# jsdjayanga/kmer-counter

Measured on NVIDIA B200. Metric: k-mers counted/s at k=31, higher is better.
Workload: dtype u64

## Files before the change

kmer-counter_b200/csrc/kc_super.cu:

```cuda
#include <math.h>
#include <stdlib.h>

#include "kc_internal.h"
#include "kc_super.cuh"

namespace kc {

namespace {

constexpr uint32_t kNoBin = 0xffffffffu;
constexpr int kSwThreads = 256;
constexpr int kSwMaxSeg = 18;
constexpr int kNb1Max = 1024;
constexpr int kRsBins = 2048;

template <uint32_t X> struct ILog2 { static constexpr uint32_t v = 1 + ILog2<(X >> 1)>::v; };
template <> struct ILog2<1> { static constexpr uint32_t v = 0; };

__host__ __device__ __forceinline__ uint32_t mmer_hash(uint32_t mm) {
    uint32_t h = mm * 0x9E3779B1u;
    h ^= h >> 15;
    h *= 0x85EBCA6Bu;
    return h;
}
__device__ __forceinline__ uint32_t bin_of_min(uint32_t mn, uint32_t n_bins) {
    return __umulhi(mn * 0xC2B2AE35u, n_bins);
}

struct SwScatterParams {
    ExtractParams ep;
    uint32_t m, w, nh, nh_stride, seg_len, segs_per_read, cmax, span;
    uint32_t h_off, bin_off, bits_off;
    uint32_t n_bins, bin_cap;
    uint64_t ovf_cap;
    uint32_t *cursor;
    uint8_t *bins;
    uint8_t *ovf;
    unsigned long long *sc;
};

template <int W, bool CANON>
__global__ void __launch_bounds__(kSwThreads) sw_scatter_kernel(SwScatterParams q) {
    const ExtractParams &p = q.ep;
    extern __shared__ __align__(128) uint8_t smem[];
    const uint32_t stage_bytes = p.stage_bytes;
    uint8_t *stage0 = smem;
    uint64_t *enc = reinterpret_cast<uint64_t *>(smem + p.enc_off);
    uint8_t *enc_b = reinterpret_cast<uint8_t *>(enc);
    const uint32_t enc_row = p.nw + 1;
    uint8_t *bad4 = smem + p.bad_off;
    uint8_t *flag = smem + p.flag_off;
    uint64_t *bars = reinterpret_cast<uint64_t *>(smem + p.bar_off);
    uint32_t *hh = reinterpret_cast<uint32_t *>(smem + q.h_off);
    uint32_t *bid = reinterpret_cast<uint32_t *>(smem + q.bin_off);
    uint32_t *seg_st = reinterpret_cast<uint32_t *>(smem + q.bits_off);
    uint32_t *seg_bd = seg_st + p.tile_reads * q.segs_per_read;
    __shared__ uint32_t s_nstart;
    const uint32_t tid = threadIdx.x, lane = tid & 31;

    if (tid == 0) {
        s_nstart = 0;
        mbar_init(&bars[0], 1);
        mbar_init(&bars[1], 1);
        mbar_fence_init();
    }
    for (uint32_t i = tid; i < p.tile_reads * enc_row; i += kSwThreads) enc[i] = 0;
    for (uint32_t i = tid; i < p.tile_reads; i += kSwThreads) flag[i] = 0;
    __syncthreads();

    auto tile_reads_of = [&](uint32_t t) -> uint32_t {
        uint64_t first = (uint64_t)t * p.tile_reads;
        uint64_t left = p.n_reads - first;
        return left < p.tile_reads ? (uint32_t)left : p.tile_reads;
    };
    auto issue_load = [&](uint32_t t, uint32_t s) {
        uint32_t bytes = tile_reads_of(t) * p.L;
        const uint8_t *src = p.reads + (uint64_t)t * p.tile_reads * p.L;
        uint8_t *dst = stage0 + s * stage_bytes;
        if ((bytes & 15u) == 0) {
            if (tid == 0) {
                asm volatile("fence.proxy.async.shared::cta;" ::: "memory");
                mbar_expect_tx(&bars[s], bytes);
                tma_load_1d(dst, src, bytes, &bars[s]);
            }
        } else {
            for (uint32_t i = tid; i < bytes; i += kSwThreads) dst[i] = src[i];
        }
    };

    uint32_t phase_bits = 0, stage = 0;
    unsigned long long invalid_local = 0, windows_local = 0, records_local = 0;
    const uint32_t mmask = q.m >= 16 ? 0xffffffffu : ((1u << (2 * q.m)) - 1u);
    const uint32_t mshift = 64 - 2 * q.m;
    const uint32_t ng = (q.nh + 7) >> 3;

    uint32_t tile = blockIdx.x;
    if (tile < p.n_tiles) issue_load(tile, 0);

    for (; tile < p.n_tiles; tile += gridDim.x) {
        const uint32_t next = tile + gridDim.x;
        if (next < p.n_tiles) issue_load(next, stage ^ 1);
        const uint32_t nreads = tile_reads_of(tile);
        if (((nreads * p.L) & 15u) == 0) {
            mbar_wait(&bars[stage], (phase_bits >> stage) & 1u);
            phase_bits ^= 1u << stage;
        } else {
            __syncthreads();
        }
        const uint8_t *src_tile = stage0 + stage * stage_bytes;

        encode_tile(p, src_tile, nreads, enc_b, bad4, flag);
        __syncthreads();
        if (tid == 0) s_nstart = 0;

        for (uint32_t g = tid; g < nreads * ng; g += kSwThreads) {
            const uint32_t r = g / ng, j0 = (g - r * ng) * 8;
            const uint32_t wi = j0 >> 5, sh = (j0 & 31u) * 2u;
            const uint64_t *e = enc + r * enc_row;
            const uint64_t a = wi <= p.nw ? e[wi] : 0ull;
            const uint64_t b = wi + 1 <= p.nw ? e[wi + 1] : 0ull;
            const uint64_t x = sh ? ((a << sh) | (b >> (64 - sh))) : a;
            uint32_t *row = hh + r * q.nh_stride + j0;
            if constexpr (CANON) {
#pragma unroll
                for (uint32_t i = 0; i < 8; i++) {
                    const uint32_t mm = (uint32_t)(x >> (mshift - 2 * i)) & mmask;
                    uint32_t r = __brev(mm);
                    r = ((r >> 1) & 0x55555555u) | ((r & 0x55555555u) << 1);
                    if (j0 + i < q.nh) row[i] = mmer_hash(min(mm, (r >> (32 - 2 * q.m)) ^ mmask));
                }
            } else {
#pragma unroll
                for (uint32_t i = 0; i < 8; i++)
                    if (j0 + i < q.nh) row[i] = mmer_hash((uint32_t)(x >> (mshift - 2 * i)) & mmask);
            }
        }
        __syncthreads();

        const uint32_t n_seg = nreads * q.segs_per_read;
        for (uint32_t sg = tid; sg < n_seg; sg += kSwThreads) {
            const uint32_t r = sg / q.segs_per_read;
            const uint32_t p0 = (sg - r * q.segs_per_read) * q.seg_len;
            if (p0 >= p.nk) { seg_st[sg] = 0; seg_bd[sg] = 0; continue; }
            const uint32_t s = min(q.seg_len, p.nk - p0);
            const uint32_t lb = p0 > 0 ? 1u : 0u;
            const uint32_t se = s + lb;
            const uint32_t *g = hh + r * q.nh_stride + p0 - lb;
            uint32_t S[kSwMaxSeg];
            S[kSwMaxSeg - 1] = 0xffffffffu;
#pragma unroll
            for (int i = kSwMaxSeg - 2; i >= 0; i--) {
                const uint32_t v = (uint32_t)i + 1 < se ? g[i] : 0xffffffffu;
                S[i] = min(v, S[i + 1]);
            }
            uint32_t core = 0xffffffffu;
            for (uint32_t t = se - 1; t < q.w; t++) core = min(core, g[t]);
            uint32_t pm = 0xffffffffu;
            const bool check = flag[r] != 0;
            uint32_t *brow = bid + r * p.nk + p0 - lb;
            uint32_t prev = kNoBin, stm = 0, bdm = 0;
#pragma unroll
            for (uint32_t i = 0; i < (uint32_t)kSwMaxSeg; i++) {
                if (i < se) {
                    const uint32_t mn = min(min(S[i], core), pm);
                    const bool valid = check ? kmer_window_valid(bad4 + r * p.nb4, p0 - lb + i, p.k) : true;
                    const uint32_t b = valid ? bin_of_min(mn, q.n_bins) : kNoBin;
                    if (i >= lb) {
                        if (!valid) invalid_local++;
                        brow[i] = b;
                        const uint32_t st = (valid && b != prev) ? 1u : 0u;
                        stm |= st << (i - lb);
                        bdm |= (st | (valid ? 0u : 1u)) << (i - lb);
                    }
                    prev = b;
                    if (i + 1 < se) pm = min(pm, g[q.w + i]);
                }
            }
            seg_st[sg] = stm;
            seg_bd[sg] = bdm;
        }
        __syncthreads();

        uint32_t *list = hh;
        for (uint32_t base = 0; base < n_seg; base += kSwThreads) {
            const uint32_t sg = base + tid;
            uint32_t stm = sg < n_seg ? seg_st[sg] : 0u;
            const uint32_t cnt = __popc(stm);
            uint32_t incl = cnt;
#pragma unroll
            for (int o = 1; o < 32; o <<= 1) {
                const uint32_t t = __shfl_up_sync(0xffffffffu, incl, o);
                if (lane >= (uint32_t)o) incl += t;
            }
            uint32_t off = 0;
            if (lane == 31 && incl) off = atomicAdd(&s_nstart, incl);
            off = __shfl_sync(0xffffffffu, off, 31) + incl - cnt;
            while (stm) {
                const uint32_t i = __ffs(stm) - 1;
                stm &= stm - 1;
                list[off++] = (sg << 5) | i;
            }
        }
        __syncthreads();
        const uint32_t n_start = s_nstart;
        for (uint32_t en = tid; en < n_start; en += kSwThreads) {
            const uint32_t ent = list[en];
            const uint32_t sg = ent >> 5, wi0 = ent & 31u;
            const uint32_t r = sg / q.segs_per_read, si = sg - r * q.segs_per_read;
            const uint32_t pos = si * q.seg_len + wi0;
            uint32_t end = p.nk;
            {
                uint32_t mk = seg_bd[sg] & ~(0xffffffffu >> (31 - wi0));
                uint32_t sj = si;
                while (mk == 0 && ++sj < q.segs_per_read) mk = seg_bd[r * q.segs_per_read + sj];
                if (mk) end = min(p.nk, sj * q.seg_len + (uint32_t)__ffs(mk) - 1);
            }
            const uint32_t len = end - pos;
            const uint32_t b = bid[r * p.nk + pos];
            const uint64_t *e = enc + r * enc_row;
            for (uint32_t q0 = 0; q0 < len; q0 += q.cmax) {
                const uint32_t idx = atomicAdd(&q.cursor[b], 1u);
                const uint32_t c = min(q.cmax, len - q0);
                const uint32_t wi = (pos + q0) >> 5, sh = ((pos + q0) & 31u) * 2u;
                uint64_t ew[2 * W + 1];
#pragma unroll
                for (int t = 0; t < 2 * W + 1; t++) ew[t] = wi + t <= p.nw ? e[wi + t] : 0ull;
                uint64_t rec[2 * W];
#pragma unroll
                for (int t = 0; t < 2 * W; t++) rec[t] = sh ? ((ew[t] << sh) | (ew[t + 1] >> (64 - sh))) : ew[t];
                const uint32_t nbases = q.span + c - 1;
#pragma unroll
                for (int t = 0; t < 2 * W; t++) {
                    const int keep = (int)nbases - 32 * t;
                    if (keep <= 0) rec[t] = 0;
                    else if (keep < 32) rec[t] &= ~0ull << (64 - 2 * keep);
                }
                rec[2 * W - 1] = (rec[2 * W - 1] & ~0xffull) | c;
                ulonglong2 *dst = nullptr;
                if (idx < q.bin_cap) {
                    dst = reinterpret_cast<ulonglong2 *>(q.bins) + ((uint64_t)b * q.bin_cap + idx) * W;
                } else {
                    const unsigned long long oi = atomicAdd(&q.sc[SW_OVF], 1ull);
                    if (oi < q.ovf_cap) dst = reinterpret_cast<ulonglong2 *>(q.ovf) + oi * W;
                    else atomicOr(&q.sc[SW_FAIL], 1ull);
                }
                if (dst) {
#pragma unroll
                    for (int t = 0; t < W; t++) dst[t] = make_ulonglong2(rec[2 * t], rec[2 * t + 1]);
                }
                windows_local += c;
                records_local++;
            }
        }
        for (uint32_t i = tid; i < nreads; i += kSwThreads) flag[i] = 0;
        __syncthreads();
        stage ^= 1;
    }
#pragma unroll
    for (int o = 16; o > 0; o >>= 1) {
        invalid_local += __shfl_xor_sync(0xffffffffu, invalid_local, o);
        windows_local += __shfl_xor_sync(0xffffffffu, windows_local, o);
        records_local += __shfl_xor_sync(0xffffffffu, records_local, o);
    }
    if (lane == 0) {
        if (invalid_local) atomicAdd(&q.sc[SW_INVALID], invalid_local);
        if (windows_local) atomicAdd(&q.sc[SW_WINDOWS], windows_local);
        if (records_local) atomicAdd(&q.sc[SW_RECORDS], records_local);
    }
}

template <int W> __device__ __forceinline__ bool key_all_ones(const Key<W> &k) {
    uint64_t a = ~0ull;
#pragma unroll
    for (int i = 0; i < W; i++) a &= k.w[i];
    return a == ~0ull;
}
template <int W> __device__ __forceinline__ bool key_any_word_ones(const Key<W> &k) {
    bool r = false;
#pragma unroll
    for (int i = 0; i < W; i++) r = r || (k.w[i] == ~0ull);
    return r;
}
template <int W> __device__ __forceinline__ void key_set_ones(Key<W> &k) {
#pragma unroll
    for (int i = 0; i < W; i++) k.w[i] = ~0ull;
}
__device__ __forceinline__ Key<1> slot_claim(Key<1> *slot, const Key<1> &k) {
    Key<1> o;
    o.w[0] = atomicCAS(reinterpret_cast<unsigned long long *>(slot), ~0ull, (unsigned long long)k.w[0]);
    return o;
}
__device__ __forceinline__ Key<2> slot_claim(Key<2> *slot, const Key<2> &k) {
    Key<2> o;
    const uint32_t a = smem_u32(slot);
    asm volatile(
        "{\n"
        ".reg .b128 c, n, o;\n"
        "mov.b128 c, {%3, %3};\n"
        "mov.b128 n, {%4, %5};\n"
        "atom.shared.cas.b128 o, [%2], c, n;\n"
        "mov.b128 {%0, %1}, o;\n"
        "}\n"
        : "=l"(o.w[0]), "=l"(o.w[1])
        : "r"(a), "l"(~0ull), "l"(k.w[0]), "l"(k.w[1])
        : "memory");
    return o;
}
template <int W> __device__ __forceinline__ uint32_t key_hash(const Key<W> &k) {
    uint32_t x = (uint32_t)k.w[0] ^ (uint32_t)(k.w[0] >> 29);
    if constexpr (W > 1) x ^= ((uint32_t)k.w[W - 1] ^ (uint32_t)(k.w[W - 1] >> 31)) * 0x85EBCA6Bu;
    return x * 0x9E3779B1u;
}
__device__ __forceinline__ uint32_t pass_hash(uint32_t h) { return (h ^ (h >> 15)) * 0x2C1B3C6Du; }

enum {
    SWP_UNIT = 0,
    SWP_DEDUP,
    SWP_SCAN,
    SWP_OPEN,
    SWP_INSERT,
    SWP_DRAIN,
    SWP_ROUND_END,
    SWP_EMIT,
    SWP_PHASES,
    SWP_QUEUED = SWP_PHASES,
    SWP_DRAIN_PROBES,
    SWP_WARPS,
    SWP_TOTAL,
    SWP_SLOTS
};
#ifdef KC_SW_PROFILE
__device__ unsigned long long g_sw_prof[SWP_SLOTS];
#define SWP_DECL                                                                                      \
    __shared__ unsigned long long s_prof[THREADS / 32][SWP_SLOTS];                                    \
    if (lane == 0)                                                                                    \
        for (int i_ = 0; i_ < SWP_SLOTS; i_++) s_prof[warp][i_] = 0;                                  \
    const long long swp_t0 = clock64();                                                               \
    long long swp_t = swp_t0
#define SWP_MARK(ph)                                                                                  \
    do {                                                                                              \
        const long long t_ = clock64();                                                               \
        if (lane == 0) s_prof[warp][ph] += (unsigned long long)(t_ - swp_t);                          \
        swp_t = t_;                                                                                   \
    } while (0)
#define SWP_ADD(c, v) atomicAdd(&s_prof[warp][c], (unsigned long long)(v))
#define SWP_ADD_ACTIVE(c)                                                                             \
    do {                                                                                              \
        const uint32_t am_ = __activemask();                                                          \
        if (lane == (uint32_t)__ffs(am_) - 1) SWP_ADD(c, __popc(am_));                                \
    } while (0)
#define SWP_FLUSH()                                                                                   \
    do {                                                                                              \
        __syncwarp();                                                                                 \
        if (lane == 0) {                                                                              \
            s_prof[warp][SWP_WARPS] = 1;                                                              \
            s_prof[warp][SWP_TOTAL] = (unsigned long long)(clock64() - swp_t0);                       \
            for (int i_ = 0; i_ < SWP_SLOTS; i_++) atomicAdd(&g_sw_prof[i_], s_prof[warp][i_]);       \
        }                                                                                             \
    } while (0)
#else
#define SWP_DECL do {} while (0)
#define SWP_MARK(ph) do {} while (0)
#define SWP_ADD(c, v) do {} while (0)
#define SWP_ADD_ACTIVE(c) do {} while (0)
#define SWP_FLUSH() do {} while (0)
#endif

struct SwCountParams {
    uint32_t n_src;
    const uint32_t *src_cursor[8];
    const uint8_t *src_bins[8];
    const unsigned long long *src_sc[8];
    uint32_t bin_begin;
    const uint8_t *ovf;
    uint32_t n_bins, bin_cap, ovf_slice;
    uint64_t ovf_cap;
    uint64_t last_mask;
    uint64_t *d_keys;
    uint32_t *d_counts;
    uint64_t d_cap;
    uint32_t *hist1;
    int shift1, nb1;
    int add_phantom;
    unsigned long long *sc;
};

template <int W, int THREADS, int TSLOTS, int RPT, bool CANON = false>
__global__ void __launch_bounds__(THREADS) sw_count_kernel(SwCountParams p) {
    constexpr int RB = THREADS * RPT;
    extern __shared__ __align__(16) uint8_t cs_smem[];
    Key<W> *tk = reinterpret_cast<Key<W> *>(cs_smem);
    ulonglong2 *recs = reinterpret_cast<ulonglong2 *>(tk + TSLOTS);
    uint32_t *tc = reinterpret_cast<uint32_t *>(recs + RB * W);
    uint32_t *s_start = tc + TSLOTS;
    uint32_t *s_hist = s_start + THREADS;
    constexpr int kQueue = RPT > 1 ? 64 : 96;
    Key<W> *queue = reinterpret_cast<Key<W> *>(s_hist + kNb1Max);
    uint32_t *queue_m = reinterpret_cast<uint32_t *>(queue + (THREADS / 32) * kQueue);
    constexpr bool DEDUP = (W == 1);
    constexpr int RT = DEDUP ? (RPT > 1 ? RB : 2 * RB) : 1;
    ulonglong2 *rt_keys = reinterpret_cast<ulonglong2 *>(queue_m + (THREADS / 32) * kQueue);
    uint32_t *rt_mult = reinterpret_cast<uint32_t *>(rt_keys + RT);
    uint32_t *rec_mult = rt_mult + RT;
    __shared__ uint32_t s_unit, s_m, s_ones, s_abort;
    __shared__ unsigned long long s_base;
    __shared__ uint32_t s_warp[THREADS / 32];
    const uint32_t tid = threadIdx.x, lane = tid & 31, warp = tid >> 5;
    constexpr uint32_t kLimit = TSLOTS / 4 * 3;
    constexpr uint32_t hshift = 32 - ILog2<(uint32_t)TSLOTS>::v;
    [[maybe_unused]] const uint32_t rc_sh = CANON ? rc_shift_of(p.last_mask) : 0u;

    {
        Key<W> empty;
        key_set_ones<W>(empty);
        for (uint32_t i = tid; i < (uint32_t)TSLOTS; i += THREADS) { tk[i] = empty; tc[i] = 0; }
        for (uint32_t i = tid; i < (uint32_t)p.nb1; i += THREADS) s_hist[i] = 0;
        if constexpr (DEDUP)
            for (uint32_t i = tid; i < (uint32_t)RT; i += THREADS) { rt_keys[i] = make_ulonglong2(~0ull, ~0ull); rt_mult[i] = 0; }
        if (tid == 0) { s_m = 0; s_ones = 0; s_abort = 0; }
    }
    unsigned long long n_ovf = p.sc[SW_OVF];
// ... 1228 lines not shown
inline uint64_t round512(uint64_t b) { return (b + 511) & ~511ull; }

constexpr int kFinCapSmall = 2048, kFinCapLarge = 4096;
constexpr int kFinCapWide = 1024;

}

static void plan_layout(SuperPlan &pl, bool ext_e);

bool super_plan(uint32_t k, uint32_t L, uint32_t flags, uint64_t max_windows, uint32_t occ_per_bin, SuperPlan *out,
                double record_headroom, uint64_t distinct_hint, bool ext_e) {
    if (k == 0 || k > 64 || L < k || L > 4096) return false;
    if (flags & kPlanCanonical) flags |= kPlanStrict;
    const bool strict = (flags & kPlanStrict) != 0;
    SuperPlan pl{};
    pl.flags = flags & (kPlanStrict | kPlanCanonical);
    pl.W = (int)((k + 31) / 32);
    pl.k = k;
    pl.L = L;
    const uint32_t mm = k % 32;
    const bool masked = strict ? (mm != 0) : (mm >= 1 && mm <= 28);
    pl.span = masked ? k : 32u * pl.W;
    pl.last_mask = masked ? (~0ull << (64 - 2 * mm)) : ~0ull;
    if (pl.span < 22) return false;
    pl.nk = L - k + 1;
    pl.cmax = 32u * pl.W - 3;
    if (max_windows == 0) max_windows = 1;
    if (occ_per_bin == 0) {
        occ_per_bin = 8192;
        if (distinct_hint && distinct_hint < max_windows) {
            const double per_key = (double)max_windows / (double)distinct_hint;
            const double occ = 2200.0 * per_key;
            if (occ < 8192.0) occ_per_bin = occ < 1024.0 ? 1024u : ((uint32_t)occ + 255u) & ~255u;
        }
    }
    uint64_t nb = (max_windows + occ_per_bin - 1) / occ_per_bin;
    if (nb < 8) nb = 8;
    if (nb > (1ull << 24)) nb = 1ull << 24;
    pl.n_bins = (uint32_t)nb;
    pl.m = 12;
    while (pl.m < 16 && pl.m + 8 < pl.span && (1ull << (2 * pl.m)) < 192ull * pl.n_bins) pl.m++;
    pl.w = pl.span - pl.m + 1;
    pl.nh = pl.nk + pl.w - 1;
    pl.nh_stride = (pl.nh + 8) | 1u;
    pl.seg_len = pl.w - 1 < (uint32_t)kSwMaxSeg - 1 ? pl.w - 1 : (uint32_t)kSwMaxSeg - 1;
    pl.segs_per_read = (pl.nk + pl.seg_len - 1) / pl.seg_len;
    pl.seg_len = (pl.nk + pl.segs_per_read - 1) / pl.segs_per_read;
    const double rho = 2.0 / (pl.w + 1) + 1.2 / pl.nk + 1.0 / pl.cmax * 0.25;
    const double est_total = (double)max_windows * rho;
    const double per_bin = est_total / (double)pl.n_bins;
    pl.bin_cap = (uint32_t)(per_bin * (1.0 + 90.0 / sqrt((double)occ_per_bin))) + 64;
    pl.bin_cap = (pl.bin_cap + 3) & ~3u;
    pl.ovf_cap = (uint64_t)(est_total * 0.6) + 8192;
    if (pl.ovf_cap < max_windows / 16) pl.ovf_cap = max_windows / 16;
    pl.ovf_slice = 4096;
    const uint64_t d_base = distinct_hint && distinct_hint < max_windows ? distinct_hint + distinct_hint / 8 + 4096 : max_windows;
    pl.d_cap = d_base + (uint64_t)((double)d_base * record_headroom) + (record_headroom > 0 ? 8192 : 0);
    if (pl.d_cap > (1ull << 32) - 2) pl.d_cap = (1ull << 32) - 2;
    if (pl.d_cap < 1024) pl.d_cap = 1024;
    pl.fin_cap = pl.d_cap > (uint64_t)kSuperMaxSub * (kFinCapSmall * 7 / 10) ? kFinCapLarge : kFinCapSmall;
    pl.sub_target = pl.fin_cap * 7 / 10;
    if (const char *v = getenv("KC_SW_SUB_TARGET")) {
        const int t = atoi(v);
        if (t > 0) pl.sub_target = (uint32_t)t;
    }
    const int sig = pl.W == 1 ? (masked ? (int)(2 * mm) : 64) : 64;
    pl.b1 = sig < 10 ? sig : 10;
    plan_layout(pl, ext_e);
    *out = pl;
    return true;
}

static void plan_layout(SuperPlan &pl, bool ext_e) {
    uint64_t o = 0;
    auto take = [&](uint64_t bytes) { uint64_t r = o; o += round512(bytes); return r; };
    const uint64_t rec_bytes = 16ull * pl.W;
    pl.off_cursor = take((uint64_t)pl.n_bins * 4);
    pl.off_hist1 = take((kNb1Max + 8) * 4);
    pl.off_hist2 = take((uint64_t)(2 * kSuperMaxSub + 8) * 4);
    pl.off_base1 = take((kNb1Max + 8) * 4);
    pl.off_cur1 = take((kNb1Max + 8) * 4);
    pl.off_base2 = take((uint64_t)(kSuperMaxSub + 8) * 4);
    pl.off_cur2 = take((uint64_t)(kSuperMaxSub + 8) * 4);
    pl.off_mout = take((uint64_t)(kSuperMaxSub + 8) * 4);
    pl.off_off = take((uint64_t)(kSuperMaxSub + 8) * 4);
    pl.off_plan = take(sizeof(SuperPlanDev));
    pl.off_x = take(sizeof(XDev));
    pl.off_sc = take(SW_COUNT * 8);
    pl.off_h2m = take((uint64_t)(kSuperMaxSub + 8) * 4);
    pl.off_big = take((uint64_t)(kSuperMaxSub + 8) * 4);
    pl.off_bigoff = take((uint64_t)(kSuperMaxSub + 8) * 4);
    pl.off_bins = take((uint64_t)pl.n_bins * pl.bin_cap * rec_bytes);
    pl.off_ovf = take(pl.ovf_cap * rec_bytes);
    pl.off_dk = take(pl.d_cap * 8 * pl.W + 64);
    pl.off_dc = take(pl.d_cap * 4 + 64);
    pl.ext_e = ext_e;
    pl.ext_ek = nullptr;
    pl.ext_ec = nullptr;
    pl.off_ek = pl.off_ec = o;
    if (!ext_e) {
        pl.off_ek = take(pl.d_cap * 8 * pl.W + 64);
        pl.off_ec = take(pl.d_cap * 4 + 64);
    }
    pl.ws_bytes = o;
}

bool place_plan(uint32_t k, bool strict, uint64_t n_records, SuperPlan *out) {
    if (k == 0 || k > 128 || n_records == 0 || n_records > (1ull << 32) - 2) return false;
    SuperPlan pl{};
    pl.W = (int)((k + 31) / 32);
    pl.k = k;
    const uint32_t mm = k % 32;
    const bool masked = strict ? (mm != 0) : (mm >= 1 && mm <= 28);
    pl.span = masked ? k : 32u * pl.W;
    pl.last_mask = masked ? (~0ull << (64 - 2 * mm)) : ~0ull;
    pl.n_bins = 8;
    pl.d_cap = n_records < 1024 ? 1024 : n_records;
    pl.fin_cap = pl.W >= 3 && n_records <= (uint64_t)kSuperMaxSub * (kFinCapWide * 7 / 10) ? kFinCapWide : kFinCapSmall;
    pl.sub_target = pl.fin_cap * 7 / 10;
    if (const char *v = getenv("KC_SW_SUB_TARGET")) {
        const int t = atoi(v);
        if (t > 0) pl.sub_target = (uint32_t)t;
    }
    const int sig = pl.W == 1 ? (masked ? (int)(2 * mm) : 64) : 64;
    pl.b1 = sig < 10 ? sig : 10;
    plan_layout(pl, false);
    *out = pl;
    return true;
}

namespace {
template <class T> T *at(void *ws, uint64_t off) { return reinterpret_cast<T *>(static_cast<uint8_t *>(ws) + off); }
uint64_t *ek_of(const SuperPlan &pl, void *ws) { return pl.ext_e ? pl.ext_ek : at<uint64_t>(ws, pl.off_ek); }
uint32_t *ec_of(const SuperPlan &pl, void *ws) { return pl.ext_e ? pl.ext_ec : at<uint32_t>(ws, pl.off_ec); }
}

cudaError_t super_reset(const SuperPlan &pl, void *ws, unsigned long long *d_sc, cudaStream_t s) {
    cudaError_t e;
    if ((e = cudaMemsetAsync(ws, 0, pl.off_base1, s)) != cudaSuccess) return e;
    return cudaMemsetAsync(d_sc, 0, SW_COUNT * 8, s);
}

template <int W>
static cudaError_t super_scatter_w(const SuperPlan &pl, const void *d_reads, uint64_t n_reads, void *ws,
                                   unsigned long long *d_sc, int n_sms, cudaStream_t s) {
    static int tile_bytes = -1;
    if (tile_bytes < 0) { const char *v = getenv("KC_SW_STAGE"); tile_bytes = v ? atoi(v) : 4800; }
    SwScatterParams q{};
    if (!extract_plan(d_reads, n_reads, pl.L, pl.k, pl.flags, &d_sc[SW_INVALID], &q.ep, (uint32_t)tile_bytes))
        return cudaErrorInvalidValue;
    if (q.ep.n_tiles == 0) return cudaSuccess;
    q.m = pl.m; q.w = pl.w; q.nh = pl.nh; q.nh_stride = pl.nh_stride;
    q.seg_len = pl.seg_len; q.segs_per_read = pl.segs_per_read; q.cmax = pl.cmax; q.span = pl.span;
    q.h_off = (q.ep.smem_total + 15u) & ~15u;
    q.bin_off = q.h_off + q.ep.tile_reads * pl.nh_stride * 4;
    q.bits_off = q.bin_off + q.ep.tile_reads * pl.nk * 4;
    const uint32_t smem = q.bits_off + 2 * q.ep.tile_reads * pl.segs_per_read * 4;
    if (smem > 200 * 1024) return cudaErrorInvalidValue;
    q.n_bins = pl.n_bins; q.bin_cap = pl.bin_cap; q.ovf_cap = pl.ovf_cap;
    q.cursor = at<uint32_t>(ws, pl.off_cursor);
    q.bins = at<uint8_t>(ws, pl.off_bins);
    q.ovf = at<uint8_t>(ws, pl.off_ovf);
    q.sc = d_sc;
    auto kern = (pl.flags & kPlanCanonical) ? sw_scatter_kernel<W, true> : sw_scatter_kernel<W, false>;
    cudaError_t e = cudaFuncSetAttribute(kern, cudaFuncAttributeMaxDynamicSharedMemorySize, (int)smem);
    if (e != cudaSuccess) return e;
    int per_sm = 1;
    cudaOccupancyMaxActiveBlocksPerMultiprocessor(&per_sm, kern, kSwThreads, smem);
    per_sm = per_sm < 1 ? 1 : (per_sm > 6 ? 6 : per_sm);
    uint32_t grid = (uint32_t)n_sms * per_sm;
    if (grid > q.ep.n_tiles) grid = q.ep.n_tiles;
    kern<<<grid, kSwThreads, smem, s>>>(q);
    return cudaGetLastError();
}

static bool super_scatter_fits(const SuperPlan &pl) {
    ExtractParams ep;
    if (!extract_plan(nullptr, 16, pl.L, pl.k, 0u, nullptr, &ep, 6400)) return false;
    const uint64_t smem = ((ep.smem_total + 15u) & ~15u) + (uint64_t)ep.tile_reads * pl.nh_stride * 4 +
                          (uint64_t)ep.tile_reads * pl.nk * 4 + 2ull * ep.tile_reads * pl.segs_per_read * 4;
    return smem <= 200 * 1024;
}

cudaError_t super_scatter(const SuperPlan &pl, const void *d_reads, uint64_t n_reads, void *ws,
                          unsigned long long *d_sc, int n_sms, cudaStream_t s) {
    if (pl.W == 1) return super_scatter_w<1>(pl, d_reads, n_reads, ws, d_sc, n_sms, s);
    if (pl.W == 2) return super_scatter_w<2>(pl, d_reads, n_reads, ws, d_sc, n_sms, s);
    return cudaErrorInvalidValue;
}

template <int W, int THREADS, int TSLOTS, int RPT = 2, bool CANON = false>
static cudaError_t launch_count(const SwCountParams &cp, int n_sms, cudaStream_t s) {
    const uint32_t RB = THREADS * RPT, RT = W == 1 ? (RPT > 1 ? RB : 2 * RB) : 1;
    const uint32_t smem = TSLOTS * (8 * W + 4) + RB * 16 * W + THREADS * 4 + kNb1Max * 4 +
                          (THREADS / 32) * (RPT > 1 ? 64 : 96) * (8 * W + 4) + RT * 20 + RB * 4 + 64;
    auto kern = sw_count_kernel<W, THREADS, TSLOTS, RPT, CANON>;
    cudaError_t e = cudaFuncSetAttribute(kern, cudaFuncAttributeMaxDynamicSharedMemorySize, (int)smem);
    if (e != cudaSuccess) return e;
    int per_sm = 1;
    cudaOccupancyMaxActiveBlocksPerMultiprocessor(&per_sm, kern, THREADS, smem);
    if (per_sm < 1) per_sm = 1;
    kern<<<(uint32_t)n_sms * per_sm, THREADS, smem, s>>>(cp);
    return cudaGetLastError();
}

template <int W>
static cudaError_t super_count_bins_w(const SuperPlan &pl, bool add_phantom, void *ws, unsigned long long *d_sc, int n_sms,
                                      cudaStream_t s, void *const *peer_ws = nullptr, uint32_t rank = 0,
                                      uint32_t n_ranks = 1) {
    cudaError_t e;
    SwCountParams cp{};
    const uint32_t n_src = peer_ws ? n_ranks : 1u;
    cp.n_src = n_src;
    for (uint32_t i = 0; i < n_src; i++) {
        void *w = peer_ws ? peer_ws[i] : ws;
        cp.src_cursor[i] = at<uint32_t>(w, pl.off_cursor);
        cp.src_bins[i] = at<uint8_t>(w, pl.off_bins);
        cp.src_sc[i] = peer_ws ? at<unsigned long long>(w, pl.off_sc) : d_sc;
    }
    cp.bin_begin = peer_ws ? (uint32_t)((uint64_t)pl.n_bins * rank / n_ranks) : 0u;
    cp.n_bins = peer_ws ? (uint32_t)((uint64_t)pl.n_bins * (rank + 1) / n_ranks) - cp.bin_begin : pl.n_bins;
    cp.ovf = at<uint8_t>(ws, pl.off_ovf);
    cp.bin_cap = pl.bin_cap; cp.ovf_slice = pl.ovf_slice; cp.ovf_cap = pl.ovf_cap;
    cp.last_mask = pl.last_mask;
    cp.d_keys = at<uint64_t>(ws, pl.off_dk); cp.d_counts = at<uint32_t>(ws, pl.off_dc); cp.d_cap = pl.d_cap;
    cp.hist1 = at<uint32_t>(ws, pl.off_hist1); cp.shift1 = 64 - pl.b1; cp.nb1 = 1 << pl.b1;
    cp.add_phantom = add_phantom ? 1 : 0;
    cp.sc = d_sc;
    if (pl.flags & kPlanCanonical) return W == 1 ? launch_count<1, 512, 4096, 2, true>(cp, n_sms, s)
                                                 : launch_count<2, 512, 4096, 1, true>(cp, n_sms, s);
    static int variant = -1;
    if (variant < 0) { const char *v = getenv("KC_SW_COUNT"); variant = v ? atoi(v) : 0; }
    if constexpr (W == 1) {
        switch (variant) {
            case 1: e = launch_count<1, 256, 2048, 2>(cp, n_sms, s); break;
            case 2: e = launch_count<1, 512, 4096, 1>(cp, n_sms, s); break;
            case 3: e = launch_count<1, 512, 8192, 1>(cp, n_sms, s); break;
            case 4: e = launch_count<1, 128, 4096, 2>(cp, n_sms, s); break;
            case 5: e = launch_count<1, 128, 2048, 2>(cp, n_sms, s); break;
            case 6: e = launch_count<1, 256, 4096, 1>(cp, n_sms, s); break;
            case 7: e = launch_count<1, 256, 4096, 4>(cp, n_sms, s); break;
            case 8: e = launch_count<1, 512, 4096, 1>(cp, n_sms, s); break;
            case 9: e = launch_count<1, 384, 4096, 2>(cp, n_sms, s); break;
            case 10: e = launch_count<1, 256, 4096, 2>(cp, n_sms, s); break;
            default: e = launch_count<1, 512, 4096, 2>(cp, n_sms, s); break;
        }
    } else {
        switch (variant) {
            case 1: e = launch_count<2, 256, 2048, 1>(cp, n_sms, s); break;
            case 2: e = launch_count<2, 256, 4096, 1>(cp, n_sms, s); break;
            case 3: e = launch_count<2, 256, 4096, 2>(cp, n_sms, s); break;
            default: e = launch_count<2, 512, 4096, 1>(cp, n_sms, s); break;
        }
    }
    return e;
}

cudaError_t super_count_bins(const SuperPlan &pl, bool add_phantom, void *ws, unsigned long long *d_sc, int n_sms,
                             cudaStream_t s, void *const *peer_ws, uint32_t rank, uint32_t n_ranks) {
    if (peer_ws && (n_ranks == 0 || n_ranks > 8 || rank >= n_ranks)) return cudaErrorInvalidValue;
    if (pl.W == 1) return super_count_bins_w<1>(pl, add_phantom, ws, d_sc, n_sms, s, peer_ws, rank, n_ranks);
    if (pl.W == 2) return super_count_bins_w<2>(pl, add_phantom, ws, d_sc, n_sms, s, peer_ws, rank, n_ranks);
    return cudaErrorInvalidValue;
}

template <int W>
static cudaError_t super_place_w(const SuperPlan &pl, void *ws, unsigned long long *d_sc, int n_sms, cudaStream_t s,
                                 cudaEvent_t *evs) {
    cudaError_t e;
    uint64_t *dk = at<uint64_t>(ws, pl.off_dk), *ek = ek_of(pl, ws);
    uint32_t *dc = at<uint32_t>(ws, pl.off_dc), *ec = ec_of(pl, ws);
    if (!ek || !ec) return cudaErrorInvalidValue;
    uint32_t *hist1 = at<uint32_t>(ws, pl.off_hist1), *base1 = at<uint32_t>(ws, pl.off_base1),
             *cur1 = at<uint32_t>(ws, pl.off_cur1), *hist2 = at<uint32_t>(ws, pl.off_hist2),
             *base2 = at<uint32_t>(ws, pl.off_base2), *cur2 = at<uint32_t>(ws, pl.off_cur2);
    SuperPlanDev *plan = at<SuperPlanDev>(ws, pl.off_plan);
    const int sig = pl.W == 1 ? 64 - (int)__builtin_ctzll(pl.last_mask ? pl.last_mask : 1) : 64;
    sw_plan_kernel<<<1, 1024, 0, s>>>(hist1, pl.b1, pl.d_cap, pl.sub_target, sig, base1, cur1, plan, d_sc);
    const uint32_t rs_smem = RsCfg<W>::TILE * (8 * W + 4) + 3 * kRsBinsPadded * 4;
    auto k1 = rec_scatter_kernel<W, 1>;
    auto k2 = rec_scatter_kernel<W, 2>;
    if ((e = cudaFuncSetAttribute(k1, cudaFuncAttributeMaxDynamicSharedMemorySize, (int)rs_smem)) != cudaSuccess) return e;
    if ((e = cudaFuncSetAttribute(k2, cudaFuncAttributeMaxDynamicSharedMemorySize, (int)rs_smem)) != cudaSuccess) return e;
    int per_sm = 1;
    cudaOccupancyMaxActiveBlocksPerMultiprocessor(&per_sm, k1, kRsThreads, rs_smem);
    if (per_sm < 1) per_sm = 1;
    const uint32_t grid = (uint32_t)n_sms * per_sm;
    k1<<<grid, kRsThreads, rs_smem, s>>>(dk, dc, ek, ec, plan, pl.b1, &d_sc[SW_D], pl.d_cap, cur1, nullptr);
    if ((e = cudaGetLastError()) != cudaSuccess) return e;
    if (evs) cudaEventRecord(evs[0], s);
    rec_hist2_kernel<W><<<(uint32_t)n_sms * 8, 256, 0, s>>>(ek, plan, hist2);
    sw_scan_kernel<<<(kSuperMaxSub + kScanTile - 1) / kScanTile, 1024, 0, s>>>(hist2, &plan->n_sub, 0, base2, cur2, nullptr);
    if ((e = cudaGetLastError()) != cudaSuccess) return e;
    if (evs) cudaEventRecord(evs[1], s);
    k2<<<grid, kRsThreads, rs_smem, s>>>(ek, ec, dk, dc, plan, pl.b1, &d_sc[SW_D], pl.d_cap, cur2, nullptr);
    if ((e = cudaGetLastError()) != cudaSuccess) return e;
    if (evs) cudaEventRecord(evs[2], s);
    return cudaSuccess;
}

cudaError_t super_place(const SuperPlan &pl, void *ws, unsigned long long *d_sc, int n_sms, cudaStream_t s, cudaEvent_t *evs) {
    if (pl.W == 1) return super_place_w<1>(pl, ws, d_sc, n_sms, s, evs);
    if (pl.W == 2) return super_place_w<2>(pl, ws, d_sc, n_sms, s, evs);
    if (pl.W == 3) return super_place_w<3>(pl, ws, d_sc, n_sms, s, evs);
    if (pl.W == 4) return super_place_w<4>(pl, ws, d_sc, n_sms, s, evs);
    return cudaErrorInvalidValue;
// ... 87 lines not shown
        if (pl.W == 3) return super_finish_w<3, true, 256, kFinCapWide>(pl, ws, d_sc, out_keys, out_counts, n_sms, s);
        if (pl.W == 4) return super_finish_w<4, true, 256, kFinCapWide>(pl, ws, d_sc, out_keys, out_counts, n_sms, s);
    } else {
        if (pl.W == 3) return super_finish_w<3, true, 512, kFinCapSmall>(pl, ws, d_sc, out_keys, out_counts, n_sms, s);
        if (pl.W == 4) return super_finish_w<4, true, 512, kFinCapSmall>(pl, ws, d_sc, out_keys, out_counts, n_sms, s);
    }
    return cudaErrorInvalidValue;
}

cudaError_t super_big_gather(const SuperPlan &pl, void *ws, uint64_t *tk, uint32_t *tc, int n_sms, cudaStream_t s) {
    SuperPlanDev *plan = at<SuperPlanDev>(ws, pl.off_plan);
    uint32_t *big = at<uint32_t>(ws, pl.off_big), *bigoff = at<uint32_t>(ws, pl.off_bigoff), *base2 = at<uint32_t>(ws, pl.off_base2);
    sw_scan_kernel<<<(kSuperMaxSub + kScanTile - 1) / kScanTile, 1024, 0, s>>>(big, &plan->n_sub, 0, bigoff, nullptr, nullptr);
    const uint64_t *dk = at<uint64_t>(ws, pl.off_dk);
    const uint32_t *dc = at<uint32_t>(ws, pl.off_dc);
    if (pl.W == 1) big_gather_kernel<1><<<(uint32_t)n_sms * 8, 256, 0, s>>>(dk, dc, base2, big, bigoff, plan, tk, tc);
    else if (pl.W == 2) big_gather_kernel<2><<<(uint32_t)n_sms * 8, 256, 0, s>>>(dk, dc, base2, big, bigoff, plan, tk, tc);
    else if (pl.W == 3) big_gather_kernel<3><<<(uint32_t)n_sms * 8, 256, 0, s>>>(dk, dc, base2, big, bigoff, plan, tk, tc);
    else big_gather_kernel<4><<<(uint32_t)n_sms * 8, 256, 0, s>>>(dk, dc, base2, big, bigoff, plan, tk, tc);
    return cudaGetLastError();
}

cudaError_t super_big_place(const SuperPlan &pl, bool dup, void *ws, unsigned long long *d_sc, const uint64_t *sk,
                            const uint32_t *sc_counts, uint64_t *out_keys, uint32_t *out_counts, int n_sms, cudaStream_t s) {
    const SuperPlanDev *plan = at<SuperPlanDev>(ws, pl.off_plan);
    const uint32_t *big = at<uint32_t>(ws, pl.off_big), *bigoff = at<uint32_t>(ws, pl.off_bigoff), *base2 = at<uint32_t>(ws, pl.off_base2);
    uint32_t *m_out = at<uint32_t>(ws, pl.off_mout);
    const uint32_t grid = (uint32_t)n_sms * 8;
    if (pl.W == 1) {
        if (dup) big_place_kernel<1, true><<<grid, 256, 0, s>>>(sk, sc_counts, base2, big, bigoff, plan, out_keys, out_counts, m_out, d_sc);
        else big_place_kernel<1, false><<<grid, 256, 0, s>>>(sk, sc_counts, base2, big, bigoff, plan, out_keys, out_counts, m_out, d_sc);
    } else if (pl.W == 2) {
        if (dup) big_place_kernel<2, true><<<grid, 256, 0, s>>>(sk, sc_counts, base2, big, bigoff, plan, out_keys, out_counts, m_out, d_sc);
        else big_place_kernel<2, false><<<grid, 256, 0, s>>>(sk, sc_counts, base2, big, bigoff, plan, out_keys, out_counts, m_out, d_sc);
    } else if (pl.W == 3 && dup) {
        big_place_kernel<3, true><<<grid, 256, 0, s>>>(sk, sc_counts, base2, big, bigoff, plan, out_keys, out_counts, m_out, d_sc);
    } else if (pl.W == 4 && dup) {
        big_place_kernel<4, true><<<grid, 256, 0, s>>>(sk, sc_counts, base2, big, bigoff, plan, out_keys, out_counts, m_out, d_sc);
    } else {
        return cudaErrorInvalidValue;
    }
    return cudaGetLastError();
}

cudaError_t super_fold_offsets(const SuperPlan &pl, void *ws, unsigned long long *d_sc, cudaStream_t s) {
    SuperPlanDev *plan = at<SuperPlanDev>(ws, pl.off_plan);
    sw_scan_kernel<<<(kSuperMaxSub + kScanTile - 1) / kScanTile, 1024, 0, s>>>(
        at<uint32_t>(ws, pl.off_mout), &plan->n_sub, 0, at<uint32_t>(ws, pl.off_off), nullptr, &d_sc[SW_OUT]);
    return cudaGetLastError();
}

cudaError_t super_gather(const SuperPlan &pl, void *ws, const uint64_t *tmp_keys, const uint32_t *tmp_counts,
                         uint64_t *out_keys, uint32_t *out_counts, int n_sms, cudaStream_t s) {
    const SuperPlanDev *plan = at<SuperPlanDev>(ws, pl.off_plan);
    const uint32_t *src = at<uint32_t>(ws, pl.off_base2), *off = at<uint32_t>(ws, pl.off_off);
    if (pl.W == 1) sw_gather_kernel<1><<<(uint32_t)n_sms * 8, 256, 0, s>>>(tmp_keys, tmp_counts, src, off, plan, out_keys, out_counts);
    else if (pl.W == 2) sw_gather_kernel<2><<<(uint32_t)n_sms * 8, 256, 0, s>>>(tmp_keys, tmp_counts, src, off, plan, out_keys, out_counts);
    else if (pl.W == 3) sw_gather_kernel<3><<<(uint32_t)n_sms * 8, 256, 0, s>>>(tmp_keys, tmp_counts, src, off, plan, out_keys, out_counts);
    else sw_gather_kernel<4><<<(uint32_t)n_sms * 8, 256, 0, s>>>(tmp_keys, tmp_counts, src, off, plan, out_keys, out_counts);
    return cudaGetLastError();
}

bool super_supported(const SuperPlan &pl) { return super_scatter_fits(pl); }

void super_use_large_finish(SuperPlan *pl) { pl->fin_cap = kFinCapLarge; }

template <int W>
static cudaError_t super_x_local_w(const SuperPlan &pl, void *ws, unsigned long long *d_sc, const uint32_t *d_all_hist,
                                   uint32_t rank, uint32_t n_ranks, bool keep_ranges, void *const *peer_ws, int n_sms,
                                   cudaStream_t s) {
    cudaError_t e;
    if (pl.ext_e) return cudaErrorInvalidValue;
    uint64_t *dk = at<uint64_t>(ws, pl.off_dk), *ek = at<uint64_t>(ws, pl.off_ek);
    uint32_t *dc = at<uint32_t>(ws, pl.off_dc), *ec = at<uint32_t>(ws, pl.off_ec);
    SuperPlanDev *plan = at<SuperPlanDev>(ws, pl.off_plan);
    const int sig = pl.W == 1 ? 64 - (int)__builtin_ctzll(pl.last_mask ? pl.last_mask : 1) : 64;
    XScalars xs{};
    for (uint32_t i = 0; i < n_ranks; i++) xs.sc[i] = peer_ws ? at<unsigned long long>(peer_ws[i], pl.off_sc) : d_sc;
    x_plan_kernel<<<1, 1024, 0, s>>>(d_all_hist, rank, n_ranks, keep_ranges ? 1 : 0, pl.d_cap, pl.sub_target,
                                     pl.fin_cap == kFinCapLarge ? 1 : 0, sig, at<uint32_t>(ws, pl.off_base1),
                                     at<uint32_t>(ws, pl.off_cur1), plan, at<XDev>(ws, pl.off_x), d_sc, xs);
    const uint32_t rs_smem = RsCfg<W>::TILE * (8 * W + 4) + 3 * kRsBinsPadded * 4;
    auto k1 = rec_scatter_kernel<W, 1>;
    if ((e = cudaFuncSetAttribute(k1, cudaFuncAttributeMaxDynamicSharedMemorySize, (int)rs_smem)) != cudaSuccess) return e;
    int per_sm = 1;
    cudaOccupancyMaxActiveBlocksPerMultiprocessor(&per_sm, k1, kRsThreads, rs_smem);
    if (per_sm < 1) per_sm = 1;
    k1<<<(uint32_t)n_sms * per_sm, kRsThreads, rs_smem, s>>>(dk, dc, ek, ec, plan, pl.b1, &d_sc[SW_D], pl.d_cap,
                                                            at<uint32_t>(ws, pl.off_cur1), nullptr);
    rec_hist2_kernel<W><<<(uint32_t)n_sms * 8, 256, 0, s>>>(ek, plan, at<uint32_t>(ws, pl.off_hist2));
    return cudaGetLastError();
}

cudaError_t super_x_local(const SuperPlan &pl, void *ws, unsigned long long *d_sc, const uint32_t *d_all_hist,
                          uint32_t rank, uint32_t n_ranks, bool keep_ranges, void *const *peer_ws, int n_sms, cudaStream_t s) {
    if (pl.b1 != kXB1 || n_ranks == 0 || n_ranks > 8 || rank >= n_ranks) return cudaErrorInvalidValue;
    if (pl.W == 1) return super_x_local_w<1>(pl, ws, d_sc, d_all_hist, rank, n_ranks, keep_ranges, peer_ws, n_sms, s);
    if (pl.W == 2) return super_x_local_w<2>(pl, ws, d_sc, d_all_hist, rank, n_ranks, keep_ranges, peer_ws, n_sms, s);
    return cudaErrorInvalidValue;
}

template <int W>
static cudaError_t super_x_pull_w(const SuperPlan &pl, void *ws, unsigned long long *d_sc, void *const *peer_ws,
                                  uint32_t rank, uint32_t n_ranks, int n_sms, cudaStream_t s) {
    cudaError_t e;
    SuperPlanDev *plan = at<SuperPlanDev>(ws, pl.off_plan);
    XDev *x = at<XDev>(ws, pl.off_x);
    XPeers peers{};
    for (uint32_t i = 0; i < n_ranks; i++) {
        peers.keys[i] = at<uint64_t>(peer_ws[i], pl.off_ek);
        peers.counts[i] = at<uint32_t>(peer_ws[i], pl.off_ec);
        peers.hist2[i] = at<uint32_t>(peer_ws[i], pl.off_hist2);
    }
    uint32_t *h2m = at<uint32_t>(ws, pl.off_h2m), *base2 = at<uint32_t>(ws, pl.off_base2), *cur2 = at<uint32_t>(ws, pl.off_cur2);
    x_merge_hist_kernel<<<(uint32_t)n_sms * 4, 256, 0, s>>>(peers, n_ranks, plan, h2m);
    sw_scan_kernel<<<(kSuperMaxSub + kScanTile - 1) / kScanTile, 1024, 0, s>>>(h2m, &plan->n_sub, 0, base2, cur2, nullptr);
    const uint32_t rs_smem = RsCfg<W>::TILE * (8 * W + 4) + 3 * kRsBinsPadded * 4;
    auto k2 = rec_scatter_kernel<W, 2>;
    if ((e = cudaFuncSetAttribute(k2, cudaFuncAttributeMaxDynamicSharedMemorySize, (int)rs_smem)) != cudaSuccess) return e;
    int per_sm = 1;
    cudaOccupancyMaxActiveBlocksPerMultiprocessor(&per_sm, k2, kRsThreads, rs_smem);
    if (per_sm < 1) per_sm = 1;
    for (uint32_t j = 1; j <= n_ranks; j++) {
        const uint32_t i = (rank + j) % n_ranks;
        k2<<<(uint32_t)n_sms * per_sm, kRsThreads, rs_smem, s>>>(peers.keys[i], peers.counts[i], at<uint64_t>(ws, pl.off_dk),
                                                                at<uint32_t>(ws, pl.off_dc), plan, pl.b1, &d_sc[SW_D],
                                                                pl.d_cap, cur2, &x->src_range[i][0]);
    }
    return cudaGetLastError();
}

cudaError_t super_x_pull(const SuperPlan &pl, void *ws, unsigned long long *d_sc, void *const *peer_ws, uint32_t rank,
                         uint32_t n_ranks, int n_sms, cudaStream_t s) {
    if (n_ranks == 0 || n_ranks > 8 || rank >= n_ranks) return cudaErrorInvalidValue;
    if (pl.W == 1) return super_x_pull_w<1>(pl, ws, d_sc, peer_ws, rank, n_ranks, n_sms, s);
    if (pl.W == 2) return super_x_pull_w<2>(pl, ws, d_sc, peer_ws, rank, n_ranks, n_sms, s);
    return cudaErrorInvalidValue;
}

uint32_t *super_hist1(const SuperPlan &pl, void *ws) { return at<uint32_t>(ws, pl.off_hist1); }
const SuperXInfo *super_x_info(const SuperPlan &pl, void *ws) { return at<XDev>(ws, pl.off_x); }

}

#ifdef KC_SW_PROFILE
extern "C" int kc_sw_profile_read(unsigned long long *out, int reset) {
    cudaError_t e = cudaMemcpyFromSymbol(out, kc::g_sw_prof, sizeof(kc::g_sw_prof));
    if (e == cudaSuccess && reset) {
        static const unsigned long long zero[kc::SWP_SLOTS] = {};
        e = cudaMemcpyToSymbol(kc::g_sw_prof, zero, sizeof(zero));
    }
    return e == cudaSuccess ? 0 : -1;
}
#endif
```

Before: 60.45 billion.

## Streamline sliding-window minimizer binning in scatter kernel with magic division

Replaces the integer divisions by ng and segs_per_read with precomputed multiply-high magic constants, and drops the per-element bounds check in the m-mer hashing loop (this relies on nh_stride padding). It rewrites the per-segment minimizer loop so the left boundary is handled uniformly and bins are stored only on a bin change or in reads with bad bases. The loop can also exit early for short segments, and window-validity masks are computed only for flagged reads. Compile-time profiling macros, off by default, are added as well. The risks are subtle correctness changes: brow is no longer written for unchanged bins, and the hash pass writes past nh.

```diff
diff --git a/kmer-counter_b200/csrc/kc_super.cu b/kmer-counter_b200/csrc/kc_super.cu
--- a/kmer-counter_b200/csrc/kc_super.cu
+++ b/kmer-counter_b200/csrc/kc_super.cu
@@ -27,9 +27,67 @@
     return __umulhi(mn * 0xC2B2AE35u, n_bins);
 }
 
+enum {
+    S1P_WAIT = 0,
+    S1P_ENCODE,
+    S1P_HASH,
+    S1P_MIN,
+    S1P_START,
+    S1P_EMIT,
+    S1P_CURSOR,
+    S1P_BAR,
+    S1P_PHASES,
+    S1P_TILES = S1P_PHASES,
+    S1P_RECORDS,
+    S1P_CUT,
+    S1P_FLAGGED,
+    S1P_WARPS,
+    S1P_TOTAL,
+    S1P_SLOTS
+};
+#ifdef KC_SW_PROFILE
+__device__ unsigned long long g_s1_prof[S1P_SLOTS];
+#define S1P_DECL                                                                                      \
+    __shared__ unsigned long long s1_prof[kSwThreads / 32][S1P_SLOTS];                                \
+    const uint32_t s1p_warp = threadIdx.x >> 5;                                                       \
+    if (lane == 0)                                                                                    \
+        for (int i_ = 0; i_ < S1P_SLOTS; i_++) s1_prof[s1p_warp][i_] = 0;                             \
+    const long long s1p_t0 = clock64();                                                               \
+    long long s1p_t = s1p_t0
+#define S1P_MARK(ph)                                                                                  \
+    do {                                                                                              \
+        const long long t_ = clock64();                                                               \
+        if (lane == 0) s1_prof[s1p_warp][ph] += (unsigned long long)(t_ - s1p_t);                     \
+        s1p_t = t_;                                                                                   \
+    } while (0)
+#define S1P_ADD(c, v) atomicAdd(&s1_prof[s1p_warp][c], (unsigned long long)(v))
+#define S1P_USE(x)                                                                                    \
+    do {                                                                                              \
+        uint32_t u_ = (x);                                                                            \
+        asm volatile("mov.b32 %0, %0;" : "+r"(u_));      \
+    } while (0)
+#define S1P_FLUSH()                                                                                   \
+    do {                                                                                              \
+        __syncwarp();                                                                                 \
+        if (lane == 0) {                                                                              \
+            s1_prof[s1p_warp][S1P_WARPS] = 1;                                                         \
+            s1_prof[s1p_warp][S1P_TOTAL] = (unsigned long long)(clock64() - s1p_t0);                  \
+            for (int i_ = 0; i_ < S1P_SLOTS; i_++) atomicAdd(&g_s1_prof[i_], s1_prof[s1p_warp][i_]);  \
+        }                                                                                             \
+    } while (0)
+#else
+#define S1P_DECL do {} while (0)
+#define S1P_MARK(ph) do {} while (0)
+#define S1P_ADD(c, v) do {} while (0)
+#define S1P_USE(x) do {} while (0)
+#define S1P_FLUSH() do {} while (0)
+#endif
+
 struct SwScatterParams {
     ExtractParams ep;
     uint32_t m, w, nh, nh_stride, seg_len, segs_per_read, cmax, span;
+    uint32_t ng;
+    uint32_t ng_magic, spr_magic;
     uint32_t h_off, bin_off, bits_off;
     uint32_t n_bins, bin_cap;
     uint64_t ovf_cap;
@@ -38,6 +96,13 @@
     uint8_t *ovf;
     unsigned long long *sc;
 };
+
+__host__ __device__ __forceinline__ uint32_t div_magic_of(uint32_t d) { return d == 1 ? 0u : (uint32_t)((1ull << 32) / d + 1); }
+__device__ __forceinline__ uint32_t div_small(uint32_t n, uint32_t d, uint32_t magic) {
+    if (d == 1) return n;
+    const uint32_t r = __umulhi(n, magic);
+    return r * d > n ? r - 1 : r;
+}
 
 template <int W, bool CANON>
 __global__ void __launch_bounds__(kSwThreads) sw_scatter_kernel(SwScatterParams q) {
@@ -57,6 +122,7 @@
     uint32_t *seg_bd = seg_st + p.tile_reads * q.segs_per_read;
     __shared__ uint32_t s_nstart;
     const uint32_t tid = threadIdx.x, lane = tid & 31;
+    S1P_DECL;
 
     if (tid == 0) {
         s_nstart = 0;
@@ -67,6 +133,7 @@
     for (uint32_t i = tid; i < p.tile_reads * enc_row; i += kSwThreads) enc[i] = 0;
     for (uint32_t i = tid; i < p.tile_reads; i += kSwThreads) flag[i] = 0;
     __syncthreads();
+    S1P_MARK(S1P_BAR);
 
     auto tile_reads_of = [&](uint32_t t) -> uint32_t {
         uint64_t first = (uint64_t)t * p.tile_reads;
@@ -92,7 +159,7 @@
     unsigned long long invalid_local = 0, windows_local = 0, records_local = 0;
     const uint32_t mmask = q.m >= 16 ? 0xffffffffu : ((1u << (2 * q.m)) - 1u);
     const uint32_t mshift = 64 - 2 * q.m;
-    const uint32_t ng = (q.nh + 7) >> 3;
+    const uint32_t ng = q.ng, spr = q.segs_per_read, w = q.w, n_bins = q.n_bins;
 
     uint32_t tile = blockIdx.x;
     if (tile < p.n_tiles) issue_load(tile, 0);
@@ -108,13 +175,16 @@
             __syncthreads();
         }
         const uint8_t *src_tile = stage0 + stage * stage_bytes;
+        S1P_MARK(S1P_WAIT);
 
         encode_tile(p, src_tile, nreads, enc_b, bad4, flag);
-        __syncthreads();
+        S1P_MARK(S1P_ENCODE);
+        __syncthreads();
+        S1P_MARK(S1P_BAR);
         if (tid == 0) s_nstart = 0;
 
         for (uint32_t g = tid; g < nreads * ng; g += kSwThreads) {
-            const uint32_t r = g / ng, j0 = (g - r * ng) * 8;
+            const uint32_t r = div_small(g, ng, q.ng_magic), j0 = (g - r * ng) * 8;
             const uint32_t wi = j0 >> 5, sh = (j0 & 31u) * 2u;
             const uint64_t *e = enc + r * enc_row;
             const uint64_t a = wi <= p.nw ? e[wi] : 0ull;
@@ -127,59 +197,66 @@
                     const uint32_t mm = (uint32_t)(x >> (mshift - 2 * i)) & mmask;
                     uint32_t r = __brev(mm);
                     r = ((r >> 1) & 0x55555555u) | ((r & 0x55555555u) << 1);
-                    if (j0 + i < q.nh) row[i] = mmer_hash(min(mm, (r >> (32 - 2 * q.m)) ^ mmask));
+                    row[i] = mmer_hash(min(mm, (r >> (32 - 2 * q.m)) ^ mmask));
                 }
             } else {
 #pragma unroll
-                for (uint32_t i = 0; i < 8; i++)
-                    if (j0 + i < q.nh) row[i] = mmer_hash((uint32_t)(x >> (mshift - 2 * i)) & mmask);
-            }
-        }
-        __syncthreads();
-
-        const uint32_t n_seg = nreads * q.segs_per_read;
+                for (uint32_t i = 0; i < 8; i++) row[i] = mmer_hash((uint32_t)(x >> (mshift - 2 * i)) & mmask);
+            }
+        }
+        S1P_MARK(S1P_HASH);
+        __syncthreads();
+        S1P_MARK(S1P_BAR);
+
+        const uint32_t n_seg = nreads * spr;
         for (uint32_t sg = tid; sg < n_seg; sg += kSwThreads) {
-            const uint32_t r = sg / q.segs_per_read;
-            const uint32_t p0 = (sg - r * q.segs_per_read) * q.seg_len;
+            const uint32_t r = div_small(sg, spr, q.spr_magic);
+            const uint32_t p0 = (sg - r * spr) * q.seg_len;
             if (p0 >= p.nk) { seg_st[sg] = 0; seg_bd[sg] = 0; continue; }
             const uint32_t s = min(q.seg_len, p.nk - p0);
-            const uint32_t lb = p0 > 0 ? 1u : 0u;
-            const uint32_t se = s + lb;
-            const uint32_t *g = hh + r * q.nh_stride + p0 - lb;
+            const uint32_t se = s + 1;
+            const uint32_t *g = hh + r * q.nh_stride + p0 - 1;
             uint32_t S[kSwMaxSeg];
             S[kSwMaxSeg - 1] = 0xffffffffu;
 #pragma unroll
             for (int i = kSwMaxSeg - 2; i >= 0; i--) {
-                const uint32_t v = (uint32_t)i + 1 < se ? g[i] : 0xffffffffu;
+                const uint32_t v = (uint32_t)i + 1 < se && (i || p0) ? g[i] : 0xffffffffu;
                 S[i] = min(v, S[i + 1]);
             }
             uint32_t core = 0xffffffffu;
-            for (uint32_t t = se - 1; t < q.w; t++) core = min(core, g[t]);
-            uint32_t pm = 0xffffffffu;
+            for (uint32_t t = se - 1; t < w; t++) core = min(core, g[t]);
             const bool check = flag[r] != 0;
-            uint32_t *brow = bid + r * p.nk + p0 - lb;
-            uint32_t prev = kNoBin, stm = 0, bdm = 0;
-#pragma unroll
-            for (uint32_t i = 0; i < (uint32_t)kSwMaxSeg; i++) {
-                if (i < se) {
-                    const uint32_t mn = min(min(S[i], core), pm);
-                    const bool valid = check ? kmer_window_valid(bad4 + r * p.nb4, p0 - lb + i, p.k) : true;
-                    const uint32_t b = valid ? bin_of_min(mn, q.n_bins) : kNoBin;
-                    if (i >= lb) {
-                        if (!valid) invalid_local++;
-                        brow[i] = b;
-                        const uint32_t st = (valid && b != prev) ? 1u : 0u;
-                        stm |= st << (i - lb);
-                        bdm |= (st | (valid ? 0u : 1u)) << (i - lb);
-                    }
-                    prev = b;
-                    if (i + 1 < se) pm = min(pm, g[q.w + i]);
-                }
-            }
-            seg_st[sg] = stm;
-            seg_bd[sg] = bdm;
-        }
-        __syncthreads();
+            uint32_t *brow = bid + r * p.nk + p0 - 1;
+            uint32_t prev = p0 ? bin_of_min(min(S[0], core), n_bins) : kNoBin;
+            uint32_t pm = 0xffffffffu, chg = 0;
+#pragma unroll
+            for (uint32_t i = 1; i < (uint32_t)kSwMaxSeg; i++) {
+                if (i >= 5 && (i & 1) && i >= se) break;
+                const bool in = i < se;
+                pm = min(pm, in ? g[w + i - 1] : 0xffffffffu);
+                const uint32_t b = bin_of_min(min(min(S[i], core), pm), n_bins);
+                const bool d = b != prev;
+                if (in && (d || check)) brow[i] = b;
+                if (d) chg |= 1u << i;
+                prev = b;
+            }
+            chg &= (2u << s) - 1u;
+            uint32_t stm = chg, bdm = chg;
+            if (check) {
+                uint32_t vm = p0 ? 0u : 1u;
+                for (uint32_t i = p0 ? 0u : 1u; i < se; i++)
+                    if (kmer_window_valid(bad4 + r * p.nb4, p0 - 1 + i, p.k)) vm |= 1u << i;
+                const uint32_t own = ((1u << se) - 1u) & ~1u;
+                stm = vm & (chg | ~(vm << 1));
+                bdm = stm | (~vm & own);
+                invalid_local += __popc(~vm & own);
+            }
+            seg_st[sg] = stm >> 1;
+            seg_bd[sg] = bdm >> 1;
+        }
+        S1P_MARK(S1P_MIN);
+        __syncthreads();
+        S1P_MARK(S1P_BAR);
 
         uint32_t *list = hh;
         for (uint32_t base = 0; base < n_seg; base += kSwThreads) {
@@ -201,18 +278,20 @@
                 list[off++] = (sg << 5) | i;
             }
         }
-        __syncthreads();
+        S1P_MARK(S1P_START);
+        __syncthreads();
+        S1P_MARK(S1P_BAR);
         const uint32_t n_start = s_nstart;
         for (uint32_t en = tid; en < n_start; en += kSwThreads) {
             const uint32_t ent = list[en];
             const uint32_t sg = ent >> 5, wi0 = ent & 31u;
-            const uint32_t r = sg / q.segs_per_read, si = sg - r * q.segs_per_read;
+            const uint32_t r = div_small(sg, spr, q.spr_magic), si = sg - r * spr;
             const uint32_t pos = si * q.seg_len + wi0;
             uint32_t end = p.nk;
             {
                 uint32_t mk = seg_bd[sg] & ~(0xffffffffu >> (31 - wi0));
                 uint32_t sj = si;
-                while (mk == 0 && ++sj < q.segs_per_read) mk = seg_bd[r * q.segs_per_read + sj];
+                while (mk == 0 && ++sj < spr) mk = seg_bd[r * spr + sj];
                 if (mk) end = min(p.nk, sj * q.seg_len + (uint32_t)__ffs(mk) - 1);
             }
             const uint32_t len = end - pos;
@@ -236,6 +315,10 @@
                     else if (keep < 32) rec[t] &= ~0ull << (64 - 2 * keep);
                 }
                 rec[2 * W - 1] = (rec[2 * W - 1] & ~0xffull) | c;
+                S1P_MARK(S1P_EMIT);
+                S1P_USE(idx);
+                S1P_MARK(S1P_CURSOR);
+                if (q0) S1P_ADD(S1P_CUT, 1);
                 ulonglong2 *dst = nullptr;
                 if (idx < q.bin_cap) {
                     dst = reinterpret_cast<ulonglong2 *>(q.bins) + ((uint64_t)b * q.bin_cap + idx) * W;
@@ -252,8 +335,14 @@
                 records_local++;
             }
         }
-        for (uint32_t i = tid; i < nreads; i += kSwThreads) flag[i] = 0;
-        __syncthreads();
+        for (uint32_t i = tid; i < nreads; i += kSwThreads) {
+            if (flag[i]) S1P_ADD(S1P_FLAGGED, 1);
+            flag[i] = 0;
+        }
+        if (tid == 0) S1P_ADD(S1P_TILES, 1);
+        S1P_MARK(S1P_EMIT);
+        __syncthreads();
+        S1P_MARK(S1P_BAR);
         stage ^= 1;
     }
 #pragma unroll
@@ -267,6 +356,8 @@
         if (windows_local) atomicAdd(&q.sc[SW_WINDOWS], windows_local);
         if (records_local) atomicAdd(&q.sc[SW_RECORDS], records_local);
     }
+    if (lane == 0) S1P_ADD(S1P_RECORDS, records_local);
+    S1P_FLUSH();
 }
 
 template <int W> __device__ __forceinline__ bool key_all_ones(const Key<W> &k) {
@@ -1801,6 +1892,8 @@
     if (q.ep.n_tiles == 0) return cudaSuccess;
     q.m = pl.m; q.w = pl.w; q.nh = pl.nh; q.nh_stride = pl.nh_stride;
     q.seg_len = pl.seg_len; q.segs_per_read = pl.segs_per_read; q.cmax = pl.cmax; q.span = pl.span;
+    q.ng = (pl.nh + 7) >> 3;
+    q.ng_magic = div_magic_of(q.ng); q.spr_magic = div_magic_of(pl.segs_per_read);
     q.h_off = (q.ep.smem_total + 15u) & ~15u;
     q.bin_off = q.h_off + q.ep.tile_reads * pl.nh_stride * 4;
     q.bits_off = q.bin_off + q.ep.tile_reads * pl.nk * 4;
@@ -2194,4 +2287,12 @@
     }
     return e == cudaSuccess ? 0 : -1;
 }
+extern "C" int kc_s1_profile_read(unsigned long long *out, int reset) {
+    cudaError_t e = cudaMemcpyFromSymbol(out, kc::g_s1_prof, sizeof(kc::g_s1_prof));
+    if (e == cudaSuccess && reset) {
+        static const unsigned long long zero[kc::S1P_SLOTS] = {};
+        e = cudaMemcpyToSymbol(kc::g_s1_prof, zero, sizeof(zero));
+    }
+    return e == cudaSuccess ? 0 : -1;
+}
 #endif
```

Result: faster. 63.95 billion, median of 6 (+5.8%).
